# bdsaglam/torch-scae

Measured on AMD Instinct MI355X. Metric: images/sec SCAE fwd+bwd, MNIST 40x40 bs=128, 1/2/4/8 MI355X, higher is better.
Workload: dtype f32

## Files before the change

### include/scae_hip.h

```cpp
#ifndef SCAE_HIP_H
#define SCAE_HIP_H

#include <stdint.h>

#ifdef __cplusplus
extern "C" {
#endif

#define SCAE_ABI_VERSION 3

#define SCAE_OK 0
#define SCAE_ERR_BAD_ARG (-1)
#define SCAE_ERR_UNSUPPORTED (-2)

#define SCAE_MAX_CHANNELS 4
#define SCAE_ATTN_MAX_SET 64
#define SCAE_RENDER_MAX_TEMPLATE_ELEMS 4096

int scae_abi_version(void);
const char *scae_error_string(int code);

void *scae_launch_list_begin(void *stream);
int scae_launch_list_end(void *list);
int scae_launch_list_size(const void *list);
// ... 169 lines not shown
int scae_object_encoder_bwd_gemm_bf16(
    const float *h, const float *q, const float *wk, const float *wv, const float *presence,
    const float *gout, float *gh, float *partial, int B, int N, int O, int C,
    const scae_gemm_desc *descs, int n, int nseg, const float *const *seg_ptr,
    const int *seg_width, const int *seg_row_stride, const int64_t *seg_batch_stride,
    float *const *seg_grad, const float *trunk_presence, const float *params,
    const float *hsave, float *pg_partial, int trunk_B, int trunk_N, int D, int Din, int Dout,
    int L, int layer_norm, void *stream);


typedef struct scae_mlp_chain_layer {
  const float *w;
  int64_t w_gs;
  int ldw, K, N;
  const float *bias;
  int64_t bias_gs;
  int bias_ld;
  const float *gate;
  int64_t gate_gs, gate_bs;
  float *out;
  int64_t out_gs, out_bs;
  int relu;
} scae_mlp_chain_layer;
typedef struct scae_mlp_chain_desc {
  scae_mlp_chain_layer layer[4];
  int n_layers;
  const float *in;
  int64_t in_gs, in_bs;
  int in_dim, B, G;
  int row_tile;
  int bf16;
} scae_mlp_chain_desc;
int scae_mlp_chain_max_width(void);
int scae_mlp_chain_fwd_f32(const scae_mlp_chain_desc *desc, void *stream);
int scae_mlp_chain_bwd_f32(const scae_mlp_chain_desc *desc, void *stream);

typedef struct scae_votes_desc {
  const float *all_param;
  const float *cpr_static, *bias_cvr, *bias_caps, *bias_vote, *bias_scale;
  const float *noise_caps, *noise_vote;
  float noise_scale;
  int V, ld_param, similarity, learn_vote_scale, allow_deformations;
  float *vote, *scale, *vote_presence, *logit_caps, *logit_vote, *reg_partial;
  float *caps_presence;
  int *caps_arg;
  const float *gvote, *gscale, *gvote_presence, *glogit_caps, *glogit_vote, *greg;
  const float *gcaps_presence;
  float *gall_param, *gcpr_in, *gall_param_gated;
} scae_votes_desc;
int scae_mlp_chain_votes_fwd_f32(const scae_mlp_chain_desc *desc, const scae_votes_desc *votes,
                                 void *stream);
int scae_mlp_chain_votes_bwd_f32(const scae_mlp_chain_desc *desc, const scae_votes_desc *votes,
                                 void *stream);

int scae_gemm_bf16(const float *A, const float *B, float *C, const float *bias,
                   const float *mask, float *asum, int batch, int M, int N, int K,
                   int a_kcontig, int lda, int64_t a_batch, int b_kcontig, int ldb,
                   int64_t b_batch, int ldc, int64_t c_batch, int bias_ld, int64_t bias_batch,
                   int ldmask, int64_t mask_batch, int64_t asum_batch, int asum_ld, int relu,
                   void *stream);
int scae_gemm_pair_bf16(const scae_gemm_desc *first, const scae_gemm_desc *second, void *stream);
int scae_gemm_multi_bf16(const scae_gemm_desc *descs, int n, void *stream);
int scae_conv3x3_fwd_fold_f32(const float *in, const float *wf, const float *bias, float *out,
                              const float *post_bias, float *out_post, int B, int IH, int IW,
                              int Cin, int Cout, int stride, const scae_seed_fold_desc *fold,
                              void *stream);
// ... 9 lines not shown
                               int stride, void *stream);

int64_t scae_conv3x3_wf_floats(int Cout, int Cin);
int scae_conv3x3_relayout_f32(const float *w, float *wf, float *wd, int Cout, int Cin,
                              void *stream);

int scae_conv3x3_bf16r_supported(int B, int IH, int IW, int Cin, int Cout, int stride);
int scae_conv3x3_first_fwd_relayout_bf16(const float *img, const float *w, const float *bias,
                                         uint16_t *out_h, int B, int Cin, int IH, int IW,
                                         int Cout, int stride, int n_layers,
                                         const float *const *rw, float *const *rwf,
                                         float *const *rwd, uint16_t *const *rwfh,
                                         uint16_t *const *rwdh, const int *rCout,
                                         const int *rCin, void *stream);
int scae_cvt_bf16_batch(int n_arrays, const float *const *src, uint16_t *const *dst,
                        const int64_t *n, void *stream);
int scae_conv3x3_fwd_bf16r(const uint16_t *in, const uint16_t *wf, const float *bias,
                           uint16_t *out_h, float *out_f, const float *post_bias,
                           float *out_post, int B, int IH, int IW, int Cin, int Cout, int stride,
                           void *stream);
int scae_conv3x3_dgrad_bf16r(const uint16_t *dpre, const uint16_t *wd, const uint16_t *gate,
                             uint16_t *din_h, float *din_f, int B, int IH, int IW, int Cin,
                             int Cout, int stride, void *stream);
int scae_conv3x3_wgrad_bf16r_splits(int B, int OH, int OW, int Cin, int Cout);
int scae_conv3x3_wgrad_bf16r(const uint16_t *dpre, const uint16_t *x, float *partial, int B,
                             int IH, int IW, int Cin, int Cout, int stride, void *stream);
int scae_conv3x3_relayout_batch_f32(int n_layers, const float *const *w, float *const *wf,
                                    float *const *wd, const int *Cout, const int *Cin,
                                    void *stream);
int scae_conv3x3_first_fwd_f32(const float *img, const float *w, const float *bias,
                               float *out, int B, int Cin, int IH, int IW, int Cout,
                               int stride, void *stream);
int scae_conv3x3_first_wgrad_rows(int B, int Cout);
int scae_conv3x3_first_wgrad_f32(const float *dpre, const float *img, float *partial, int B,
                                 int Cin, int IH, int IW, int Cout, int stride, void *stream);
int scae_conv3x3_first_fwd_relayout_f32(const float *img, const float *w, const float *bias,
                                        float *out, int B, int Cin, int IH, int IW, int Cout,
                                        int stride, int n_layers, const float *const *rw,
                                        float *const *rwf, float *const *rwd, const int *rCout,
                                        const int *rCin, void *stream);
int scae_conv3x3_first_wgrad_reduce_f32(const float *dpre, const float *img, float *partial,
                                        int B, int Cin, int IH, int IW, int Cout, int stride,
                                        int n_layers, const float *const *rpartial,
                                        float *const *rdw, float *const *rdb, const int *rCout,
                                        const int *rCin, const int *rsplits, void *stream);
int scae_conv3x3_fwd_f32(const float *in, const float *wf, const float *bias, float *out,
                         const float *post_bias, float *out_post, int B, int IH, int IW,
                         int Cin, int Cout, int stride, void *stream);
int scae_conv3x3_dgrad_f32(const float *dpre, const float *wd, const float *gate, float *din,
                           int B, int IH, int IW, int Cin, int Cout, int stride, void *stream);
int scae_conv3x3_bwd_pair_f32(const float *dpre, const float *wd, const float *in, float *din,
                              float *partial, int B, int IH, int IW, int Cin, int Cout,
                              int stride, void *stream);
int scae_conv3x3_bwd_pair_reduce_f32(const float *dpre, const float *wd, const float *in,
                                     float *din, float *partial, int B, int IH, int IW, int Cin,
                                     int Cout, int stride, const float *rpartial, int rows,
                                     const float *q, const float *wk, float *gq, float *gwk,
                                     float *gbk, float *gwv, float *gbv, int O, int C,
                                     void *stream);
int scae_conv3x3_bwd_pair_fold_f32(const float *dpre, const float *wd, const float *in,
                                   float *din, float *partial, int B, int IH, int IW, int Cin,
                                   int Cout, int stride, const scae_seed_fold_desc *fold,
                                   const scae_seed_fold_grads *fold_grads, void *stream);
int scae_conv3x3_wgrad_splits(int B, int OH, int OW, int Cin, int Cout);
int scae_conv3x3_wgrad_f32(const float *dpre, const float *in, float *partial, float *dw,
                           float *db, int B, int IH, int IW, int Cin, int Cout, int stride,
// ... 657 lines not shown
```

### torch_scae_amd/_lib.py

```python
import ctypes
import os
from ctypes import (POINTER, Structure, c_char_p, c_double, c_float, c_int,
                    c_int64, c_uint32, c_uint64, c_void_p)

_HERE = os.path.dirname(os.path.abspath(__file__))
LIB_PATH = os.environ.get("SCAE_HIP_LIB") or os.path.join(_HERE, "lib",
                                                        "libscae_hip.so")

P = c_void_p


class DecoderDesc(Structure):
    _fields_ = [("templates", P), ("templates_alpha", P), ("pose", P),
                ("presence", P), ("bg_image", P), ("bg_value", P),
                ("bg_mixing_logit", P), ("temperature_logit", P),
                ("out_scale", P),
                ("B", c_int), ("M", c_int), ("C", c_int), ("th", c_int),
                ("tw", c_int), ("H", c_int), ("W", c_int),
                ("template_repeat", c_int)]


class LikelihoodBwdDesc(Structure):
    _fields_ = [(n, P) for n in (
        "vote", "scale", "vote_presence", "dummy_vote", "x", "presence",
# ... 198 lines not shown
                                              c_int, c_int64, c_int, c_int64,
                                              c_int, c_int64, c_int64, c_int, c_int,
                                              P],
    "scae_gemm_pair_f32": [POINTER(GemmDesc), POINTER(GemmDesc), P],
    "scae_launch_list_begin": [P],
    "scae_launch_list_end": [P],
    "scae_launch_list_size": [P],
    "scae_launch_list_run": [P, P],
    "scae_launch_list_lane": [P, c_int],
    "scae_launch_list_timeline": [P, P, P, POINTER(c_float), c_int],
    "scae_launch_list_free": [P],
    "scae_gemm_multi_f32": [POINTER(GemmDesc), c_int, P],
    "scae_gemm_multi_bf16": [POINTER(GemmDesc), c_int, P],
    "scae_mlp_chain_max_width": [],
    "scae_mlp_chain_fwd_f32": [POINTER(MlpChainDesc), P],
    "scae_mlp_chain_bwd_f32": [POINTER(MlpChainDesc), P],
    "scae_mlp_chain_votes_fwd_f32": [POINTER(MlpChainDesc), POINTER(VotesDesc), P],
    "scae_mlp_chain_votes_bwd_f32": [POINTER(MlpChainDesc), POINTER(VotesDesc), P],
    "scae_gemm_pair_bf16": [POINTER(GemmDesc), POINTER(GemmDesc), P],
    "scae_conv3x3_wf_floats": [c_int, c_int],
    "scae_conv3x3_relayout_f32": [P, P, P, c_int, c_int, P],
    "scae_conv3x3_bf16r_supported": [c_int] * 6,
    "scae_conv3x3_first_fwd_relayout_bf16": [P] * 4 + [c_int] * 7 + [P] * 8,
    "scae_cvt_bf16_batch": [c_int, P, P, P, P],
    "scae_conv3x3_fwd_bf16r": [P] * 7 + [c_int] * 6 + [P],
    "scae_conv3x3_dgrad_bf16r": [P] * 5 + [c_int] * 6 + [P],
    "scae_conv3x3_wgrad_bf16r_splits": [c_int] * 5,
    "scae_conv3x3_wgrad_bf16r": [P] * 3 + [c_int] * 6 + [P],
    "scae_conv3x3_relayout_batch_f32": [c_int, P, P, P, P, P, P],
    "scae_conv3x3_first_fwd_f32": [P] * 4 + [c_int] * 6 + [P],
    "scae_conv3x3_first_fwd_relayout_f32": [P] * 4 + [c_int] * 7 + [P] * 6,
    "scae_conv3x3_first_wgrad_reduce_f32": [P] * 3 + [c_int] * 7 + [P] * 7,
    "scae_conv3x3_first_wgrad_rows": [c_int] * 2,
    "scae_conv3x3_first_wgrad_f32": [P] * 3 + [c_int] * 6 + [P],
    "scae_conv3x3_fwd_f32": [P] * 6 + [c_int] * 6 + [P],
    "scae_conv3x3_fwd_fold_f32": [P] * 6 + [c_int] * 6 + [POINTER(SeedFoldDesc), P],
    "scae_conv3x3_fwd_res_supported": [c_int] * 6,
    "scae_conv3x3_fwd_res_f32": [P] * 6 + [c_int] * 7 + [P],
    "scae_conv3x3_fwd_bf16": [P] * 6 + [c_int] * 6 + [P],
    "scae_conv3x3_dgrad_f32": [P] * 4 + [c_int] * 6 + [P],
    "scae_conv3x3_bwd_pair_f32": [P] * 5 + [c_int] * 6 + [P],
    "scae_conv3x3_bwd_pair_reduce_f32": [P] * 5 + [c_int] * 6 + [P, c_int] + [P] * 7
    + [c_int] * 2 + [P],
    "scae_conv3x3_bwd_pair_fold_f32": [P] * 5 + [c_int] * 6
    + [POINTER(SeedFoldDesc), POINTER(SeedFoldGrads), P],
    "scae_conv3x3_bwd_pair_bf16": [P] * 5 + [c_int] * 6 + [P],
    "scae_conv3x3_wgrad_reduce_batch_f32": [c_int] + [P] * 7,
    "scae_conv3x3_wgrad_splits": [c_int] * 5,
    "scae_conv3x3_wgrad_f32": [P] * 5 + [c_int] * 6 + [P],
    "scae_attention_pool_supported": [c_int] * 3,
    "scae_attention_pool_fwd_f32": [P, P] + [c_int] * 4 + [P],
    "scae_attention_pool_bwd_f32": [P, P, P] + [c_int] * 4 + [P],
    "scae_stage_batch": [P, P, c_int64, P, P, c_int64, P],
    "scae_step_prologue_f32": [P, P, c_int64, P, P, c_int64, P, c_int64, P,
                               POINTER(SeedFoldDesc), P],
    "scae_step_prologue_first_f32": [P, P, c_int64, P, P, c_int64, P, c_int64,
                                     P, POINTER(SeedFoldDesc),
                                     POINTER(FirstLayerDesc), P],
    "scae_gather_batch_f32": [P, P, c_int, POINTER(BatchSourceDesc), P],
    "scae_step_prologue_source_f32": [P, P, c_int, POINTER(BatchSourceDesc), P, c_int64, P,
                                      POINTER(SeedFoldDesc), POINTER(FirstLayerDesc), P],
    "scae_rmsprop_step_f32": [P, P, P, P, c_int64, c_float, P, c_float, c_float,
                              c_float, c_float, c_float, P],
    "scae_rmsprop_sums_step_f32": [P, P, P, P, c_int64, c_float, P, c_float, c_float,
                                   c_float, c_float, POINTER(SumJob), c_int, P],
    "scae_flat_opt_step_f32": [P, P, P, P, P, c_int64, P, P, c_int, c_double, c_double, c_float,
# ... 252 lines not shown
```

### torch_scae_amd/csrc/conv_first_dev.h

```cpp
#pragma once
#include "common.h"

namespace scae_first {
struct ConvGeom {
  int B, IH, IW, OH, OW, Cin, Cout, stride;
};

struct RelayoutBatch {
  const float *w[8];
  float *wf[8], *wd[8];
  int Cout[8], Cin[8];
  unsigned short *wfh[8], *wdh[8];
};
__host__ __device__ inline unsigned short bf16_bits(float v) {
  union { float f; unsigned u; } c;
  c.f = v;
  if ((c.u & 0x7fffffffu) > 0x7f800000u) return (unsigned short)((c.u >> 16) | 0x40);
  return (unsigned short)((c.u + 0x7fffu + ((c.u >> 16) & 1u)) >> 16);
}
__host__ __device__ inline size_t packed_index(int Cin, int co, int tap, int ci, int plane) {
  const size_t chunk = (size_t)(co >> 5) * (9 * (Cin >> 5)) + tap * (Cin >> 5) + (ci >> 5);
  return ((((chunk * 2 + ((ci & 15) >> 3)) * 3 + plane) * 64 + ((ci & 31) >> 4) * 32 + (co & 31)) << 3) +
         (ci & 7);
}
// ... 26 lines not shown
  }
  if (wfh) wfh[((size_t)co * 9 + tap) * Cin + ci] = bf16_bits(v);
  if (wdh) wdh[((size_t)ci * 9 + tap) * Cout + co] = bf16_bits(v);
}
__device__ __forceinline__ void relayout_batch(const RelayoutBatch &r, int l, int e) {
  relayout_one(r.w[l], r.wf[l], r.wd[l], r.Cout[l], r.Cin[l], e, r.wfh[l], r.wdh[l]);
}
inline int fill_relayout(RelayoutBatch &r, int n_layers, const float *const *w, float *const *wf,
                         float *const *wd, const int *Cout, const int *Cin,
                         unsigned short *const *wfh = nullptr,
                         unsigned short *const *wdh = nullptr) {
  if (!(n_layers > 0 && n_layers <= 8 && w && wf && wd && Cout && Cin)) return -1;
  int nmax = 0;
  for (int l = 0; l < n_layers; ++l) {
    if (!(w[l] && wf[l] && wd[l] && Cout[l] > 0 && Cin[l] > 0)) return -1;
    r.w[l] = w[l], r.wf[l] = wf[l], r.wd[l] = wd[l], r.Cout[l] = Cout[l], r.Cin[l] = Cin[l];
    r.wfh[l] = wfh ? wfh[l] : nullptr, r.wdh[l] = wdh ? wdh[l] : nullptr;
    nmax = nmax > Cout[l] * Cin[l] * 9 ? nmax : Cout[l] * Cin[l] * 9;
  }
  return (nmax + 255) / 256;
}

struct FirstSplit {
  int nchunk, parts, slices;
};
__host__ __device__ inline FirstSplit first_split(int B, int Cout) {
  FirstSplit f;
  f.nchunk = Cout / 64;
  f.parts = (f.nchunk <= 4 && 4 % f.nchunk == 0) ? 4 / f.nchunk : 1;
  int s = (512 + B - 1) / B;
  f.slices = s < 1 ? 1 : (s > 8 ? 8 : s);
  return f;
}

__host__ __device__ inline bool first_vec(int Cout) {
  return Cout == 64 || Cout == 128 || Cout == 256;
}
__device__ __forceinline__ void stage_image(float *s_img, const float *img, int n, int count) {
  for (int e = threadIdx.x; e < count; e += 256) s_img[e] = img[(size_t)n * count + e];
  __syncthreads();
}

template <int CIN, typename Stage>
__device__ __forceinline__ void fwd_block_from(const Stage &stage,
                                               const float *__restrict__ w,
                                               const float *__restrict__ bias,
                                               float *__restrict__ out, const ConvGeom &g,
                                               int blk, float *s_img,
                                               unsigned short *__restrict__ out_h = nullptr) {
  const FirstSplit f = first_split(g.B, g.Cout);
  const int n = blk / f.slices, slice = blk % f.slices;
  const int wave = threadIdx.x >> 6, lane = threadIdx.x & 63;
  stage(s_img, n);
  const int P = g.OH * g.OW, per = (P + f.slices - 1) / f.slices;
  const int pbeg = slice * per, pend = min(P, pbeg + per);
  if (first_vec(g.Cout)) {
    const int QL = g.Cout / 4, PPW = 64 / QL, cq = lane % QL, ps = lane / QL;
    float wr[4][CIN * 9], b4[4];
#pragma unroll
    for (int c = 0; c < 4; ++c) {
#pragma unroll
      for (int k = 0; k < CIN * 9; ++k) wr[c][k] = w[(size_t)(4 * cq + c) * CIN * 9 + k];
      b4[c] = bias[4 * cq + c];
    }
    const int step = 4 * PPW;
    int p = pbeg + wave * PPW + ps;
    int oh = p / g.OW, ow = p - oh * g.OW;
    float *dst = out + ((size_t)n * P + p) * g.Cout + 4 * cq;
    unsigned short *dst_h = out_h ? out_h + ((size_t)n * P + p) * g.Cout + 4 * cq : nullptr;
    for (; p < pend; p += step) {
      const float *src = s_img + oh * g.stride * g.IW + ow * g.stride;
      float acc[4] = {b4[0], b4[1], b4[2], b4[3]};
#pragma unroll
      for (int ci = 0; ci < CIN; ++ci)
#pragma unroll
        for (int t = 0; t < 9; ++t) {
          const float x = src[(ci * g.IH + t / 3) * g.IW + t % 3];
#pragma unroll
          for (int c = 0; c < 4; ++c) acc[c] = fmaf(x, wr[c][ci * 9 + t], acc[c]);
        }
      if (dst_h) {
        const unsigned lo = bf16_bits(fmaxf(acc[0], 0.f)) | ((unsigned)bf16_bits(fmaxf(acc[1], 0.f)) << 16);
        const unsigned hi = bf16_bits(fmaxf(acc[2], 0.f)) | ((unsigned)bf16_bits(fmaxf(acc[3], 0.f)) << 16);
        *reinterpret_cast<uint2 *>(dst_h) = make_uint2(lo, hi);
        dst_h += (size_t)step * g.Cout;
      } else {
        *reinterpret_cast<float4 *>(dst) = make_float4(fmaxf(acc[0], 0.f), fmaxf(acc[1], 0.f),
// ... 48 lines not shown
```

### torch_scae_amd/csrc/conv_mfma.hip

```cpp
#include <cstdlib>

#include "mfma_tile.h"
#include "mfma_pipe.h"
#include "conv_first_dev.h"
#include "seed_fold_dev.h"

#include <algorithm>

#include "wave_mfma.h"

#define SCAE_DEVICE_ONLY
namespace scae_sf {
#include "seed_fold.hip"
}
namespace scae_saw {
#include "seed_attention_wave.hip"
}
#undef SCAE_DEVICE_ONLY

namespace {
using namespace scae_tile;

using scae_first::ConvGeom;

// ... 1152 lines not shown
extern "C" int scae_conv3x3_relayout_f32(const float *w, float *wf, float *wd, int Cout,
                                         int Cin, void *stream) {
  SCAE_REQUIRE(w && wf && wd && Cout > 0 && Cin > 0);
  const int n = Cout * Cin * 9;
  scae::launch(relayout_weights_kernel, dim3((n + 255) / 256), dim3(256), 0,
                     (hipStream_t)stream, w, wf, wd, Cout, Cin);
  return scae_launch_status();
}

using scae_first::fill_relayout;

extern "C" int scae_conv3x3_relayout_batch_f32(int n_layers, const float *const *w,
                                               float *const *wf, float *const *wd,
                                               const int *Cout, const int *Cin, void *stream) {
  RelayoutBatch r{};
  const int rb = fill_relayout(r, n_layers, w, wf, wd, Cout, Cin);
  SCAE_REQUIRE(rb > 0);
  scae::launch(relayout_batch_kernel, dim3(rb, n_layers), dim3(256), 0,
                     (hipStream_t)stream, r);
  return scae_launch_status();
}

static int first_fwd_relayout(
    const float *img, const float *w, const float *bias, float *out, unsigned short *out_h, int B,
    int Cin, int IH, int IW, int Cout, int stride, int n_layers, const float *const *rw,
    float *const *rwf, float *const *rwd, unsigned short *const *rwfh,
    unsigned short *const *rwdh, const int *rCout, const int *rCin, void *stream) {
  ConvGeom g{B, IH, IW, (IH - 3) / stride + 1, (IW - 3) / stride + 1, Cin, Cout, stride};
  int rc = check_geom(g, false);
  if (rc) return rc;
  SCAE_REQUIRE(img && w && bias && (out || out_h) && n_layers >= 0);
  if (!out) out = reinterpret_cast<float *>(out_h);
  if (Cout % 64) return SCAE_ERR_UNSUPPORTED;
  const FirstSplit f = first_split(B, Cout);
  const size_t lds = (size_t)Cin * IH * IW * sizeof(float);
  if (lds > 64 * 1024) return SCAE_ERR_UNSUPPORTED;
  RelayoutBatch r{};
  int rb = 0;
  if (n_layers > 0) {
    rb = fill_relayout(r, n_layers, rw, rwf, rwd, rCout, rCin, rwfh, rwdh);
    SCAE_REQUIRE(rb > 0);
  }
  const int n_first = B * f.slices;
#define SCAE_FIRST_FWD(CI)                                                                    \
  case CI:                                                                                    \
    scae::launch(conv_first_fwd_kernel<CI>, dim3(n_first + n_layers * rb), dim3(256),   \
                       lds, (hipStream_t)stream, img, w, bias, out, g, r, n_first, rb, out_h); \
    break;
  switch (Cin) {
    SCAE_FIRST_FWD(1) SCAE_FIRST_FWD(2) SCAE_FIRST_FWD(3) SCAE_FIRST_FWD(4)
    default: return SCAE_ERR_UNSUPPORTED;
  }
#undef SCAE_FIRST_FWD
  return scae_launch_status();
}

extern "C" int scae_conv3x3_first_fwd_relayout_f32(
    const float *img, const float *w, const float *bias, float *out, int B, int Cin, int IH,
    int IW, int Cout, int stride, int n_layers, const float *const *rw, float *const *rwf,
    float *const *rwd, const int *rCout, const int *rCin, void *stream) {
  SCAE_REQUIRE(out);
  return first_fwd_relayout(img, w, bias, out, nullptr, B, Cin, IH, IW, Cout, stride, n_layers, rw,
                            rwf, rwd, nullptr, nullptr, rCout, rCin, stream);
}
extern "C" int scae_conv3x3_first_fwd_relayout_bf16(
    const float *img, const float *w, const float *bias, uint16_t *out_h, int B, int Cin, int IH,
    int IW, int Cout, int stride, int n_layers, const float *const *rw, float *const *rwf,
    float *const *rwd, uint16_t *const *rwfh, uint16_t *const *rwdh, const int *rCout,
    const int *rCin, void *stream) {
  SCAE_REQUIRE(out_h && (n_layers == 0 || (rwfh && rwdh)));
  return first_fwd_relayout(img, w, bias, nullptr, out_h, B, Cin, IH, IW, Cout, stride, n_layers,
                            rw, rwf, rwd, rwfh, rwdh, rCout, rCin, stream);
}

extern "C" int scae_conv3x3_first_fwd_f32(const float *img, const float *w, const float *bias,
                                          float *out, int B, int Cin, int IH, int IW, int Cout,
                                          int stride, void *stream) {
  return scae_conv3x3_first_fwd_relayout_f32(img, w, bias, out, B, Cin, IH, IW, Cout, stride, 0,
                                             nullptr, nullptr, nullptr, nullptr, nullptr, stream);
}

extern "C" int scae_conv3x3_first_wgrad_rows(int B, int Cout) {
  if (B <= 0 || Cout <= 0 || Cout % 64) return 0;
  const FirstSplit f = first_split(B, Cout);
  return B * f.slices;
}

static int fill_reduce(ReduceBatch &r, int n_layers, const float *const *partial,
                       float *const *dw, float *const *db, const int *Cout, const int *Cin,
                       const int *splits) {
  if (!(n_layers > 0 && n_layers <= 8 && partial && dw && db && Cout && Cin && splits)) return -1;
  int nmax = 0;
  for (int l = 0; l < n_layers; ++l) {
    if (!(partial[l] && dw[l] && Cout[l] > 0 && Cin[l] > 0 && splits[l] > 0)) return -1;
    r.partial[l] = partial[l], r.dw[l] = dw[l], r.db[l] = db[l];
    r.Cout[l] = Cout[l], r.Cin[l] = Cin[l], r.splits[l] = splits[l];
    const int n = 9 * Cout[l] * Cin[l] + Cout[l];
    nmax = nmax > n ? nmax : n;
  }
  return (nmax + 255) / 256;
}

extern "C" int scae_conv3x3_first_wgrad_reduce_f32(
    const float *dpre, const float *img, float *partial, int B, int Cin, int IH, int IW,
    int Cout, int stride, int n_layers, const float *const *rpartial, float *const *rdw,
    float *const *rdb, const int *rCout, const int *rCin, const int *rsplits, void *stream) {
  ConvGeom g{B, IH, IW, (IH - 3) / stride + 1, (IW - 3) / stride + 1, Cin, Cout, stride};
  int rc = check_geom(g, false);
  if (rc) return rc;
  SCAE_REQUIRE(dpre && img && partial && n_layers >= 0);
  if (Cout % 64) return SCAE_ERR_UNSUPPORTED;
  const FirstSplit f = first_split(B, Cout);
  const size_t lds = ((size_t)Cin * IH * IW +
                      (f.parts > 1 ? (size_t)f.parts * Cout * (Cin * 9 + 1) : 0)) * sizeof(float);
  if (lds > 64 * 1024) return SCAE_ERR_UNSUPPORTED;
  ReduceBatch r{};
  int rb = 0;
  if (n_layers > 0) {
// ... 308 lines not shown
```

### torch_scae_amd/csrc/mlp_chain.hip

```cpp
#include "common.h"
#include "capsule_votes_dev.h"

namespace {
typedef float f32x4 __attribute__((ext_vector_type(4)));
#ifndef SCAE_CHAIN_CH
#define SCAE_CHAIN_CH 4
#endif
#ifndef SCAE_CHAIN_ABL
#define SCAE_CHAIN_ABL 0
#endif
#ifndef SCAE_CHAIN_LB4
#define SCAE_CHAIN_LB4 1
#endif
constexpr int NW = 8, NT = 64 * NW, MAXL = 4, CH = SCAE_CHAIN_CH;
constexpr int KC = 16 * CH;
constexpr int QPR = KC / 4;
constexpr int RPI = 64 / QPR;
static_assert(CH == 8 || CH == 4, "chunk widths of 128 or 64");
constexpr int WLD = KC + 4;

struct Layer {
  const float *w;
  long w_gs;
  int ldw, K, N;
  const float *bias;
  long bias_gs;
  int bias_ld;
  const float *gate;
  long gate_gs, gate_bs;
  float *out;
  long out_gs, out_bs;
  int relu, vec;
// ... 59 lines not shown
  if (ldw >= 0) return;
#endif
  if (!BWD) {
    const int o = ((n0 + lane / QPR) * ldw + k0 + 4 * (lane % QPR)) * 4;
#pragma unroll
    for (int i = 0; i < CH; ++i) buf[i] = bload4(rs, o + RPI * i * ldw * 4);
  } else {
    const int o = ((k0 + (lane >> 2)) * ldw + n0 + 4 * (lane & 3)) * 4;
#pragma unroll
    for (int i = 0; i < CH; ++i) buf[i] = bload4(rs, o + 16 * i * ldw * 4);
  }
  if (ch == nch - 1) {
    const int r = lane & 15, q = lane >> 4, col = n0 + r;
    const bool cok = col < LN;
    if (!BWD) {
      epi[0].x = L.bias ? ldg(L.bias + (size_t)g * L.bias_gs, (size_t)col * L.bias_ld, cok) : 0.f;
    } else {
#pragma unroll
      for (int rb = 0; rb < RBT; ++rb) {
        epi[rb] = make_float4(1.f, 1.f, 1.f, 1.f);
        if (L.gate) {
          const float *gp = L.gate + (size_t)g * L.gate_gs;
          const int b = b0 + 16 * rb + 4 * q;
          epi[rb].x = ldg(gp, (size_t)b * L.gate_bs + col, cok && b < B);
          epi[rb].y = ldg(gp, (size_t)(b + 1) * L.gate_bs + col, cok && b + 1 < B);
          epi[rb].z = ldg(gp, (size_t)(b + 2) * L.gate_bs + col, cok && b + 2 < B);
          epi[rb].w = ldg(gp, (size_t)(b + 3) * L.gate_bs + col, cok && b + 3 < B);
        }
      }
    }
  }
}

template <bool BWD, int RBT, bool BF>
__global__ __launch_bounds__(NT, (RBT == 1 && SCAE_CHAIN_LB4) ? 4 : 2) void chain_kernel(Chain c) {
  constexpr int RB = 16 * RBT;
  extern __shared__ __attribute__((aligned(16))) float smem[];
  const int tid = threadIdx.x, wid = __builtin_amdgcn_readfirstlane(tid >> 6), lane = tid & 63,
            r = lane & 15, q = lane >> 4;
  const int g = blockIdx.x % c.G, b0 = (blockIdx.x / c.G) * RB;
  auto buf = [&](int p) { return smem + (p ? RB * c.stride[0] : 0); };
  float *wbase = smem + RB * (c.stride[0] + c.stride[1]);
  float *wtile = wbase + wid * (16 * WLD);
  auto park = [&](const float4 (&buf4)[CH]) {
    if (!BWD) {
      float *d = wtile + (lane / QPR) * WLD + 4 * (lane % QPR);
#pragma unroll
      for (int i = 0; i < CH; ++i) *reinterpret_cast<float4 *>(d + RPI * i * WLD) = buf4[i];
    } else {
      float *d = wtile + 4 * (lane & 3) * WLD + (lane >> 2);
#pragma unroll
      for (int i = 0; i < CH; ++i) {
        d[16 * i] = buf4[i].x;
        d[WLD + 16 * i] = buf4[i].y;
        d[2 * WLD + 16 * i] = buf4[i].z;
        d[3 * WLD + 16 * i] = buf4[i].w;
      }
    }
    asm volatile("s_waitcnt lgkmcnt(0)" ::: "memory");
  };
  auto ntiles_of = [&](int li) { return (c.l[li].N + 15) >> 4; };
  auto nch_of = [&](int li) { return (((c.l[li].K + 15) >> 4) + CH - 1) / CH; };

  float4 f[CH], fe[RBT];
#pragma unroll
  for (int rb = 0; rb < RBT; ++rb) fe[rb] = make_float4(0.f, 0.f, 0.f, 0.f);
  if (wid < ntiles_of(0))
    fetch_item<BWD, RBT>(c.l[0], c.l[0].w + (size_t)g * c.l[0].w_gs, g, b0, c.B, wid, 0, nch_of(0),
// ... 144 lines not shown
    if (V <= 0 || !v->cpr_static || !v->bias_cvr || !v->bias_caps || !v->bias_vote ||
        !v->bias_scale || v->ld_param < A)
      return SCAE_ERR_BAD_ARG;
    const scae_mlp_chain_layer &e = d->layer[bwd ? 0 : d->n_layers - 1];
    if ((bwd ? d->in_dim : e.N) != A) return SCAE_ERR_BAD_ARG;
    c.votes = 1;
    c.va = scae_votes::VoteArgs{v->all_param, v->cpr_static, v->bias_cvr, v->bias_caps,
                                v->bias_vote, v->bias_scale, v->noise_caps, v->noise_vote,
                                v->noise_scale, d->B, d->G, V, v->similarity,
                                v->learn_vote_scale, v->allow_deformations, v->ld_param};
    if (!bwd) {
      if (!(v->vote && v->scale && v->vote_presence && v->logit_caps && v->logit_vote &&
            v->reg_partial) || !v->caps_presence != !v->caps_arg)
        return SCAE_ERR_BAD_ARG;
      if (e.out_gs != v->ld_param || e.out_bs != (int64_t)d->G * v->ld_param)
        return SCAE_ERR_BAD_ARG;
      c.vo = scae_votes::VoteOut{v->vote, v->scale, v->vote_presence, v->logit_caps,
                                 v->logit_vote, v->reg_partial, v->caps_presence, v->caps_arg};
    } else {
      if (!(v->all_param && v->gall_param && v->gcpr_in) ||
          (v->gcaps_presence && !v->caps_arg))
        return SCAE_ERR_BAD_ARG;
      c.vg = scae_votes::VoteGrads{v->gvote, v->gscale, v->gvote_presence, v->glogit_caps,
                                   v->glogit_vote, v->greg, v->gcaps_presence, v->caps_arg,
                                   v->gall_param, v->gcpr_in, v->gall_param_gated};
    }
  }
  return SCAE_OK;
}

#ifndef SCAE_CHAIN_RB32_MIN_WGS
#define SCAE_CHAIN_RB32_MIN_WGS 512
#endif
template <bool BWD, int RBT, bool BF>
int launch_rb_bf(const Chain &c, void *stream) {
  constexpr int RB = 16 * RBT;
  const size_t lds = ((size_t)RB * (c.stride[0] + c.stride[1]) + (size_t)NW * 16 * WLD) * sizeof(float);
  if (lds > 48 * 1024) {
    hipError_t e = hipFuncSetAttribute(reinterpret_cast<const void *>(chain_kernel<BWD, RBT, BF>),
                                       hipFuncAttributeMaxDynamicSharedMemorySize, (int)lds);
    if (e != hipSuccess) return (int)e;
  }
  const int blocks = c.G * ((c.B + RB - 1) / RB);
  scae::launch((chain_kernel<BWD, RBT, BF>), dim3(blocks), dim3(NT), lds, (hipStream_t)stream, c);
  return scae_launch_status();
}
template <bool BWD, int RBT>
int launch_rb(const Chain &c, void *stream) {
  return c.bf16 ? launch_rb_bf<BWD, RBT, true>(c, stream) : launch_rb_bf<BWD, RBT, false>(c, stream);
}

template <bool BWD>
int launch(const scae_mlp_chain_desc *d, const scae_votes_desc *v, void *stream) {
  Chain c{};
  int rc = fill(c, d, BWD, v);
  if (rc) return rc;
  const int want = d->row_tile;
  if (want != 0 && want != 16 && want != 32) return SCAE_ERR_BAD_ARG;
  Chain c2 = c;
  int dim[2] = {c.in_dim, 16};
  for (int i = 0; i < c.n; ++i)
    if (i + 1 < c.n || (!BWD && c.votes)) dim[(i + 1) & 1] = dim[(i + 1) & 1] > c.l[i].N ? dim[(i + 1) & 1] : c.l[i].N;
  c2.stride[0] = ((dim[0] + 15) & ~15) + 4, c2.stride[1] = ((dim[1] + 15) & ~15) + 4;
  const size_t lds2 = ((size_t)32 * (c2.stride[0] + c2.stride[1]) + (size_t)NW * 16 * WLD) * sizeof(float);
  const bool scratch_ok = !c.votes || (size_t)16 * c.va.V * 7 <= (size_t)NW * 16 * WLD;
  const bool big = c.G * ((c.B + 31) / 32) >= SCAE_CHAIN_RB32_MIN_WGS;
  c2.wscratch = 1;
  const size_t lds1 = ((size_t)16 * (c.stride[0] + c.stride[1]) + (size_t)NW * 16 * WLD) * sizeof(float);
  const size_t lds1n = ((size_t)16 * (c2.stride[0] + c2.stride[1]) + (size_t)NW * 16 * WLD) * sizeof(float);
  const bool narrow16 = scratch_ok && lds1 > 80 * 1024 && lds1n <= 80 * 1024;
  if (lds2 <= 160 * 1024 && scratch_ok && want != 16 && (want == 32 || (big && !narrow16)))
    return launch_rb<BWD, 2>(c2, stream);
  if (narrow16) return launch_rb<BWD, 1>(c2, stream);
  return launch_rb<BWD, 1>(c, stream);
}
}

extern "C" int scae_mlp_chain_max_width(void) { return 704; }

extern "C" int scae_mlp_chain_fwd_f32(const scae_mlp_chain_desc *desc, void *stream) {
  return launch<false>(desc, nullptr, stream);
}
extern "C" int scae_mlp_chain_bwd_f32(const scae_mlp_chain_desc *desc, void *stream) {
  return launch<true>(desc, nullptr, stream);
}
extern "C" int scae_mlp_chain_votes_fwd_f32(const scae_mlp_chain_desc *desc,
                                            const scae_votes_desc *votes, void *stream) {
  SCAE_REQUIRE(votes);
  return launch<false>(desc, votes, stream);
}
extern "C" int scae_mlp_chain_votes_bwd_f32(const scae_mlp_chain_desc *desc,
                                            const scae_votes_desc *votes, void *stream) {
  SCAE_REQUIRE(votes);
  return launch<true>(desc, votes, stream);
}
```

### torch_scae_amd/csrc/step_prologue.hip

```cpp
#include "common.h"
#include "batch_source_dev.h"
#include "noise_dev.h"
#include "seed_fold_dev.h"
#include "conv_first_dev.h"

namespace {
constexpr int NT = 256;
static_assert(scae_noise::NT == NT && scae_fold::NT == NT, "one block size for all parts");

struct Prologue {
  float *dst_image;
  const float *src_image;
  long n_image;
  int64_t *dst_label;
  const int64_t *src_label;
  long n_label;
  float *noise;
  int64_t n_noise;
  uint64_t *noise_state;
  scae_seed_fold_desc fold;
  scae_fold::Plan plan;
  const float *first_img, *first_w, *first_bias;
  float *first_out;
  unsigned short *first_out_h;
  scae_first::ConvGeom first_g;
  scae_first::RelayoutBatch rl;
  int n_first, rb;
  int nb_stage, nb_noise, nb_fold, nb_first;
  scae_batch_source_desc src;
};

template <int CIN, bool SRC>
__global__ __launch_bounds__(NT) void step_prologue_kernel(Prologue p) {
  extern __shared__ __attribute__((aligned(16))) float lds[];
  int blk = blockIdx.x;
  if (blk < p.nb_fold) {
    scae_fold::forward_block_any(p.fold, p.plan, blk, lds);
    return;
  }
  blk -= p.nb_fold;
  if (CIN > 0) {
    if (blk < p.n_first) {
      if (SRC) {
        const int B = p.nb_stage;
        const auto stage = [&](float *s, int n) {
          scae_src::gather_image(p.src, p.src.position + (int64_t)p.src.rank * B + n, s);
          __syncthreads();
        };
        scae_first::fwd_block_from<(CIN > 0 ? CIN : 1)>(stage, p.first_w, p.first_bias,
                                                        p.first_out, p.first_g, blk, lds,
                                                        p.first_out_h);
      } else {
        scae_first::fwd_block<(CIN > 0 ? CIN : 1)>(p.first_img, p.first_w, p.first_bias,
                                                   p.first_out, p.first_g, blk, lds,
                                                   p.first_out_h);
      }
      return;
    }
    if (blk < p.nb_first) {
      const int w_ = blk - p.n_first;
      scae_first::relayout_batch(p.rl, w_ / p.rb, (w_ % p.rb) * NT + threadIdx.x);
      return;
    }
    blk -= p.nb_first;
  }
  if (blk < p.nb_noise) {
    scae_noise::uniform_block(p.noise, p.n_noise, p.noise_state, blk, p.nb_noise);
    return;
  }
  blk -= p.nb_noise;
  if (SRC) {
    const int B = p.nb_stage;
    const scae_src::Draw d = scae_src::gather_image(
// ... 41 lines not shown
  } else {
    SCAE_REQUIRE(n_image == 0 && n_label == 0);
  }
  if (n_noise > 0) {
    SCAE_REQUIRE(noise && noise_state);
    p.noise = noise, p.n_noise = n_noise, p.noise_state = noise_state;
    p.nb_noise = scae_noise::blocks_for(n_noise);
  } else {
    SCAE_REQUIRE(n_noise == 0);
  }
  if (fold) {
    const scae_seed_fold_desc &a = *fold;
    SCAE_REQUIRE(a.seeds && a.wq && a.bq && a.wk && a.bk && a.wv && a.bv && a.wo && a.bo &&
                 a.w2 && a.b2 && a.q && a.wkf && a.bkf && a.wvf && a.bvf && a.wv2e);
    if (!scae_seed_fold_supported(a.O, a.C, a.D)) return SCAE_ERR_UNSUPPORTED;
    p.fold = a;
    p.plan = scae_fold::plan(a.C, a.D);
    p.nb_fold = p.plan.blocks();
    lds = scae_fold::lds_bytes(a.C, a.D);
  }
  int cin = 0;
  if (first) {
    const scae_first_layer_desc &f = *first;
    SCAE_REQUIRE((f.img || src) && f.w && f.bias && f.out && f.B > 0 && f.IH >= 3 && f.IW >= 3 &&
                 f.Cout > 0 && f.stride > 0 && f.n_layers >= 0 && f.n_layers <= 8);
    if (f.Cin < 1 || f.Cin > 4 || f.Cout % 64) return SCAE_ERR_UNSUPPORTED;
    const size_t img_lds = (size_t)f.Cin * f.IH * f.IW * sizeof(float);
    if (img_lds > 64 * 1024) return SCAE_ERR_UNSUPPORTED;
    lds = lds > img_lds ? lds : img_lds;
    p.first_img = f.img, p.first_w = f.w, p.first_bias = f.bias, p.first_out = f.out;
    p.first_out_h = f.out_h;
    p.first_g = scae_first::ConvGeom{f.B, f.IH, f.IW, (f.IH - 3) / f.stride + 1,
                                     (f.IW - 3) / f.stride + 1, f.Cin, f.Cout, f.stride};
    p.n_first = f.B * scae_first::first_split(f.B, f.Cout).slices;
    if (f.n_layers > 0) {
      p.rb = scae_first::fill_relayout(p.rl, f.n_layers, f.rw, f.rwf, f.rwd, f.rCout, f.rCin,
                                       f.out_h ? f.rwfh : nullptr, f.out_h ? f.rwdh : nullptr);
      SCAE_REQUIRE(p.rb > 0);
    }
    p.nb_first = p.n_first + f.n_layers * p.rb;
    cin = f.Cin;
  }
  const int grid = p.nb_stage + p.nb_noise + p.nb_fold + p.nb_first;
  SCAE_REQUIRE(grid > 0);
#define SCAE_PROLOGUE(CI, SRC)                                                                \
  case CI + 8 * SRC: {                                                                        \
    const void *k = reinterpret_cast<const void *>(step_prologue_kernel<CI, SRC>);            \
    if (lds > 48 * 1024) {                                                                    \
      hipError_t e = hipFuncSetAttribute(k, hipFuncAttributeMaxDynamicSharedMemorySize, (int)lds); \
      if (e != hipSuccess) return (int)e;                                                     \
    }                                                                                         \
    scae::launch(step_prologue_kernel<CI, SRC>, dim3(grid), dim3(NT), lds,                    \
                 (hipStream_t)stream, p);                                                     \
  } break;
  switch (cin + (src ? 8 : 0)) {
    SCAE_PROLOGUE(0, false) SCAE_PROLOGUE(1, false) SCAE_PROLOGUE(2, false)
    SCAE_PROLOGUE(3, false) SCAE_PROLOGUE(4, false)
    SCAE_PROLOGUE(0, true) SCAE_PROLOGUE(1, true) SCAE_PROLOGUE(2, true)
    SCAE_PROLOGUE(3, true) SCAE_PROLOGUE(4, true)
  }
#undef SCAE_PROLOGUE
  return scae_launch_status();
}
}

extern "C" int scae_step_prologue_first_f32(float *dst_image, const float *src_image,
                                            int64_t n_image, int64_t *dst_label,
                                            const int64_t *src_label, int64_t n_label,
                                            float *noise, int64_t n_noise, uint64_t *noise_state,
                                            const scae_seed_fold_desc *fold,
                                            const scae_first_layer_desc *first, void *stream) {
  return prologue_launch(dst_image, src_image, n_image, dst_label, src_label, n_label, nullptr,
                         0, noise, n_noise, noise_state, fold, first, stream);
}

extern "C" int scae_step_prologue_source_f32(float *dst_image, int64_t *dst_label, int B,
                                             const scae_batch_source_desc *src, float *noise,
                                             int64_t n_noise, uint64_t *noise_state,
                                             const scae_seed_fold_desc *fold,
                                             const scae_first_layer_desc *first, void *stream) {
  SCAE_REQUIRE(src);
  return prologue_launch(dst_image, nullptr, 0, dst_label, nullptr, 0, src, B, noise, n_noise,
                         noise_state, fold, first, stream);
}

extern "C" int scae_step_prologue_f32(float *dst_image, const float *src_image, int64_t n_image,
                                      int64_t *dst_label, const int64_t *src_label,
                                      int64_t n_label, float *noise, int64_t n_noise,
                                      uint64_t *noise_state, const scae_seed_fold_desc *fold,
                                      void *stream) {
  return scae_step_prologue_first_f32(dst_image, src_image, n_image, dst_label, src_label,
                                      n_label, noise, n_noise, noise_state, fold, nullptr, stream);
}
```

Measured before the change: 269,000.

## Tune first-conv slicing, uncap chain bwd occupancy bound, specialize lean prologue

Decouples the first-conv forward slice count from the wgrad split, targeting a fixed workgroup count (512) so small batches spread across more blocks. Adds a variant of the MLP chain backward kernel without the occupancy-4 launch bound, used when the grid fits within the CU count, so the compiler can allocate more registers. Specializes the step prologue kernel on whether a fold stage exists, removing the fold branch when it is absent. Together these add template variants and a runtime mode switch, at the cost of extra compile-time instantiations.

```diff
diff --git a/include/scae_hip.h b/include/scae_hip.h
--- a/include/scae_hip.h
+++ b/include/scae_hip.h
@@ -225,6 +225,8 @@
   int bf16;
 } scae_mlp_chain_desc;
 int scae_mlp_chain_max_width(void);
+int scae_mlp_chain_uncapped(int blocks, int cus);
+int scae_mlp_chain_budget(int mode);
 int scae_mlp_chain_fwd_f32(const scae_mlp_chain_desc *desc, void *stream);
 int scae_mlp_chain_bwd_f32(const scae_mlp_chain_desc *desc, void *stream);
 
@@ -300,6 +302,7 @@
                                float *out, int B, int Cin, int IH, int IW, int Cout,
                                int stride, void *stream);
 int scae_conv3x3_first_wgrad_rows(int B, int Cout);
+int scae_conv3x3_first_fwd_slices(int B, int Cout);
 int scae_conv3x3_first_wgrad_f32(const float *dpre, const float *img, float *partial, int B,
                                  int Cin, int IH, int IW, int Cout, int stride, void *stream);
 int scae_conv3x3_first_fwd_relayout_f32(const float *img, const float *w, const float *bias,
diff --git a/torch_scae_amd/_lib.py b/torch_scae_amd/_lib.py
--- a/torch_scae_amd/_lib.py
+++ b/torch_scae_amd/_lib.py
@@ -254,6 +254,9 @@
     "scae_conv3x3_first_fwd_relayout_f32": [P] * 4 + [c_int] * 7 + [P] * 6,
     "scae_conv3x3_first_wgrad_reduce_f32": [P] * 3 + [c_int] * 7 + [P] * 7,
     "scae_conv3x3_first_wgrad_rows": [c_int] * 2,
+    "scae_conv3x3_first_fwd_slices": [c_int] * 2,
+    "scae_mlp_chain_uncapped": [c_int] * 2,
+    "scae_mlp_chain_budget": [c_int],
     "scae_conv3x3_first_wgrad_f32": [P] * 3 + [c_int] * 6 + [P],
     "scae_conv3x3_fwd_f32": [P] * 6 + [c_int] * 6 + [P],
     "scae_conv3x3_fwd_fold_f32": [P] * 6 + [c_int] * 6 + [POINTER(SeedFoldDesc), P],
diff --git a/torch_scae_amd/csrc/conv_first_dev.h b/torch_scae_amd/csrc/conv_first_dev.h
--- a/torch_scae_amd/csrc/conv_first_dev.h
+++ b/torch_scae_amd/csrc/conv_first_dev.h
@@ -82,6 +82,17 @@
   f.slices = s < 1 ? 1 : (s > 8 ? 8 : s);
   return f;
 }
+#ifndef SCAE_FIRST_FWD_WGS
+#define SCAE_FIRST_FWD_WGS 512
+#endif
+#ifndef SCAE_FIRST_FWD_MAX_SLICES
+#define SCAE_FIRST_FWD_MAX_SLICES 8
+#endif
+__host__ __device__ inline int first_fwd_slices(int B, int Cout) {
+  (void)Cout;
+  const int s = (SCAE_FIRST_FWD_WGS + B - 1) / B;
+  return s < 1 ? 1 : (s > SCAE_FIRST_FWD_MAX_SLICES ? SCAE_FIRST_FWD_MAX_SLICES : s);
+}
 
 __host__ __device__ inline bool first_vec(int Cout) {
   return Cout == 64 || Cout == 128 || Cout == 256;
@@ -99,10 +110,11 @@
                                                int blk, float *s_img,
                                                unsigned short *__restrict__ out_h = nullptr) {
   const FirstSplit f = first_split(g.B, g.Cout);
-  const int n = blk / f.slices, slice = blk % f.slices;
+  const int slices = first_fwd_slices(g.B, g.Cout);
+  const int n = blk / slices, slice = blk % slices;
   const int wave = threadIdx.x >> 6, lane = threadIdx.x & 63;
   stage(s_img, n);
-  const int P = g.OH * g.OW, per = (P + f.slices - 1) / f.slices;
+  const int P = g.OH * g.OW, per = (P + slices - 1) / slices;
   const int pbeg = slice * per, pend = min(P, pbeg + per);
   if (first_vec(g.Cout)) {
     const int QL = g.Cout / 4, PPW = 64 / QL, cq = lane % QL, ps = lane / QL;
diff --git a/torch_scae_amd/csrc/conv_mfma.hip b/torch_scae_amd/csrc/conv_mfma.hip
--- a/torch_scae_amd/csrc/conv_mfma.hip
+++ b/torch_scae_amd/csrc/conv_mfma.hip
@@ -1208,7 +1208,6 @@
   SCAE_REQUIRE(img && w && bias && (out || out_h) && n_layers >= 0);
   if (!out) out = reinterpret_cast<float *>(out_h);
   if (Cout % 64) return SCAE_ERR_UNSUPPORTED;
-  const FirstSplit f = first_split(B, Cout);
   const size_t lds = (size_t)Cin * IH * IW * sizeof(float);
   if (lds > 64 * 1024) return SCAE_ERR_UNSUPPORTED;
   RelayoutBatch r{};
@@ -1217,8 +1216,8 @@
     rb = fill_relayout(r, n_layers, rw, rwf, rwd, rCout, rCin, rwfh, rwdh);
     SCAE_REQUIRE(rb > 0);
   }
-  const int n_first = B * f.slices;
-#define SCAE_FIRST_FWD(CI)                                                                    \
+  const int n_first = B * scae_first::first_fwd_slices(B, Cout);
+#define SCAE_FIRST_FWD(CI)                                                                   \
   case CI:                                                                                    \
     scae::launch(conv_first_fwd_kernel<CI>, dim3(n_first + n_layers * rb), dim3(256),   \
                        lds, (hipStream_t)stream, img, w, bias, out, g, r, n_first, rb, out_h); \
@@ -1260,6 +1259,11 @@
   if (B <= 0 || Cout <= 0 || Cout % 64) return 0;
   const FirstSplit f = first_split(B, Cout);
   return B * f.slices;
+}
+
+extern "C" int scae_conv3x3_first_fwd_slices(int B, int Cout) {
+  if (B <= 0 || Cout <= 0 || Cout % 64) return 0;
+  return scae_first::first_fwd_slices(B, Cout);
 }
 
 static int fill_reduce(ReduceBatch &r, int n_layers, const float *const *partial,
diff --git a/torch_scae_amd/csrc/mlp_chain.hip b/torch_scae_amd/csrc/mlp_chain.hip
--- a/torch_scae_amd/csrc/mlp_chain.hip
+++ b/torch_scae_amd/csrc/mlp_chain.hip
@@ -1,3 +1,5 @@
+#include <atomic>
+
 #include "common.h"
 #include "capsule_votes_dev.h"
 
@@ -123,8 +125,8 @@
   }
 }
 
-template <bool BWD, int RBT, bool BF>
-__global__ __launch_bounds__(NT, (RBT == 1 && SCAE_CHAIN_LB4) ? 4 : 2) void chain_kernel(Chain c) {
+template <bool BWD, int RBT, bool BF, bool CAP>
+__global__ __launch_bounds__(NT, (RBT == 1 && CAP && SCAE_CHAIN_LB4) ? 4 : 2) void chain_kernel(Chain c) {
   constexpr int RB = 16 * RBT;
   extern __shared__ __attribute__((aligned(16))) float smem[];
   const int tid = threadIdx.x, wid = __builtin_amdgcn_readfirstlane(tid >> 6), lane = tid & 63,
@@ -335,22 +337,45 @@
 #ifndef SCAE_CHAIN_RB32_MIN_WGS
 #define SCAE_CHAIN_RB32_MIN_WGS 512
 #endif
-template <bool BWD, int RBT, bool BF>
+std::atomic<int> g_budget{0};
+bool chain_uncapped(int blocks, int cus) {
+  const int mode = g_budget.load(std::memory_order_relaxed);
+  return mode == 1 ? false : (mode == 2 ? true : scae_mlp_chain_uncapped(blocks, cus) != 0);
+}
+int device_cus() {
+  static std::atomic<int> cached[64];
+  int dev = 0;
+  if (hipGetDevice(&dev) != hipSuccess || dev < 0 || dev >= 64) return 0;
+  int n = cached[dev].load(std::memory_order_relaxed);
+  if (n == 0) {
+    if (hipDeviceGetAttribute(&n, hipDeviceAttributeMultiprocessorCount, dev) != hipSuccess) n = 0;
+    cached[dev].store(n, std::memory_order_relaxed);
+  }
+  return n;
+}
+
+template <bool BWD, int RBT, bool BF, bool CAP>
 int launch_rb_bf(const Chain &c, void *stream) {
   constexpr int RB = 16 * RBT;
   const size_t lds = ((size_t)RB * (c.stride[0] + c.stride[1]) + (size_t)NW * 16 * WLD) * sizeof(float);
   if (lds > 48 * 1024) {
-    hipError_t e = hipFuncSetAttribute(reinterpret_cast<const void *>(chain_kernel<BWD, RBT, BF>),
+    hipError_t e = hipFuncSetAttribute(reinterpret_cast<const void *>(chain_kernel<BWD, RBT, BF, CAP>),
                                        hipFuncAttributeMaxDynamicSharedMemorySize, (int)lds);
     if (e != hipSuccess) return (int)e;
   }
   const int blocks = c.G * ((c.B + RB - 1) / RB);
-  scae::launch((chain_kernel<BWD, RBT, BF>), dim3(blocks), dim3(NT), lds, (hipStream_t)stream, c);
+  scae::launch((chain_kernel<BWD, RBT, BF, CAP>), dim3(blocks), dim3(NT), lds, (hipStream_t)stream, c);
   return scae_launch_status();
 }
 template <bool BWD, int RBT>
 int launch_rb(const Chain &c, void *stream) {
-  return c.bf16 ? launch_rb_bf<BWD, RBT, true>(c, stream) : launch_rb_bf<BWD, RBT, false>(c, stream);
+  if constexpr (RBT == 1 && BWD) {
+    if (chain_uncapped(c.G * ((c.B + 15) / 16), device_cus()))
+      return c.bf16 ? launch_rb_bf<BWD, RBT, true, false>(c, stream)
+                    : launch_rb_bf<BWD, RBT, false, false>(c, stream);
+  }
+  return c.bf16 ? launch_rb_bf<BWD, RBT, true, true>(c, stream)
+                : launch_rb_bf<BWD, RBT, false, true>(c, stream);
 }
 
 template <bool BWD>
@@ -381,6 +406,14 @@
 
 extern "C" int scae_mlp_chain_max_width(void) { return 704; }
 
+extern "C" int scae_mlp_chain_uncapped(int blocks, int cus) {
+  return blocks > 0 && cus > 0 && blocks <= cus;
+}
+extern "C" int scae_mlp_chain_budget(int mode) {
+  if (mode < 0 || mode > 2) return g_budget.load(std::memory_order_relaxed);
+  return g_budget.exchange(mode, std::memory_order_relaxed);
+}
+
 extern "C" int scae_mlp_chain_fwd_f32(const scae_mlp_chain_desc *desc, void *stream) {
   return launch<false>(desc, nullptr, stream);
 }
diff --git a/torch_scae_amd/csrc/step_prologue.hip b/torch_scae_amd/csrc/step_prologue.hip
--- a/torch_scae_amd/csrc/step_prologue.hip
+++ b/torch_scae_amd/csrc/step_prologue.hip
@@ -30,15 +30,17 @@
   scae_batch_source_desc src;
 };
 
-template <int CIN, bool SRC>
+template <int CIN, bool SRC, bool FOLD>
 __global__ __launch_bounds__(NT) void step_prologue_kernel(Prologue p) {
   extern __shared__ __attribute__((aligned(16))) float lds[];
   int blk = blockIdx.x;
-  if (blk < p.nb_fold) {
-    scae_fold::forward_block_any(p.fold, p.plan, blk, lds);
-    return;
-  }
-  blk -= p.nb_fold;
+  if constexpr (FOLD) {
+    if (blk < p.nb_fold) {
+      scae_fold::forward_block_any(p.fold, p.plan, blk, lds);
+      return;
+    }
+    blk -= p.nb_fold;
+  }
   if (CIN > 0) {
     if (blk < p.n_first) {
       if (SRC) {
@@ -146,7 +148,7 @@
     p.first_out_h = f.out_h;
     p.first_g = scae_first::ConvGeom{f.B, f.IH, f.IW, (f.IH - 3) / f.stride + 1,
                                      (f.IW - 3) / f.stride + 1, f.Cin, f.Cout, f.stride};
-    p.n_first = f.B * scae_first::first_split(f.B, f.Cout).slices;
+    p.n_first = f.B * scae_first::first_fwd_slices(f.B, f.Cout);
     if (f.n_layers > 0) {
       p.rb = scae_first::fill_relayout(p.rl, f.n_layers, f.rw, f.rwf, f.rwd, f.rCout, f.rCin,
                                        f.out_h ? f.rwfh : nullptr, f.out_h ? f.rwdh : nullptr);
@@ -157,23 +159,29 @@
   }
   const int grid = p.nb_stage + p.nb_noise + p.nb_fold + p.nb_first;
   SCAE_REQUIRE(grid > 0);
-#define SCAE_PROLOGUE(CI, SRC)                                                                \
-  case CI + 8 * SRC: {                                                                        \
-    const void *k = reinterpret_cast<const void *>(step_prologue_kernel<CI, SRC>);            \
+#define SCAE_PROLOGUE_(CI, SRC, FOLD)                                                         \
+  case CI + 8 * SRC + 16 * FOLD: {                                                            \
+    const void *k = reinterpret_cast<const void *>(step_prologue_kernel<CI, SRC, FOLD>);      \
     if (lds > 48 * 1024) {                                                                    \
       hipError_t e = hipFuncSetAttribute(k, hipFuncAttributeMaxDynamicSharedMemorySize, (int)lds); \
       if (e != hipSuccess) return (int)e;                                                     \
     }                                                                                         \
-    scae::launch(step_prologue_kernel<CI, SRC>, dim3(grid), dim3(NT), lds,                    \
+    scae::launch(step_prologue_kernel<CI, SRC, FOLD>, dim3(grid), dim3(NT), lds,              \
                  (hipStream_t)stream, p);                                                     \
   } break;
-  switch (cin + (src ? 8 : 0)) {
+#define SCAE_PROLOGUE(CI, SRC) SCAE_PROLOGUE_(CI, SRC, false) SCAE_PROLOGUE_(CI, SRC, true)
+#ifndef SCAE_PROLOGUE_LEAN_MAX_FIRST
+#define SCAE_PROLOGUE_LEAN_MAX_FIRST 512
+#endif
+  const bool lean = !fold && p.n_first <= SCAE_PROLOGUE_LEAN_MAX_FIRST;
+  switch (cin + (src ? 8 : 0) + (lean ? 0 : 16)) {
     SCAE_PROLOGUE(0, false) SCAE_PROLOGUE(1, false) SCAE_PROLOGUE(2, false)
     SCAE_PROLOGUE(3, false) SCAE_PROLOGUE(4, false)
     SCAE_PROLOGUE(0, true) SCAE_PROLOGUE(1, true) SCAE_PROLOGUE(2, true)
     SCAE_PROLOGUE(3, true) SCAE_PROLOGUE(4, true)
   }
 #undef SCAE_PROLOGUE
+#undef SCAE_PROLOGUE_
   return scae_launch_status();
 }
 }
```

After: 270,900, median of 6. Within noise of the previous version (+0.7%).
